# adelacvg/NS2VC

Measured on AMD Instinct MI355X. Metric: denoiser-steps/sec (10s@24kHz Vocos latent, bs32), higher is better.
Workload: dtype fp16

## Files before the change

### include/ns2vc_hip.h

```cpp
#ifndef NS2VC_HIP_H
#define NS2VC_HIP_H

#include <stddef.h>
#include <stdint.h>

#ifdef __cplusplus
extern "C" {
#endif

#define NS2VC_ABI_VERSION 7
#define NS2VC_MAX_LEVELS 8
#define NS2VC_NCOEF 12

typedef struct ns2vc_unet ns2vc_unet;

typedef struct ns2vc_unet_cfg {
  int32_t latent_channels;
  int32_t content_channels;
  int32_t n_levels;
  int32_t block_out_channels[NS2VC_MAX_LEVELS];
  int32_t norm_num_groups;
  int32_t cross_attention_dim;
  int32_t heads;
  int32_t layers_per_block;
// ... 133 lines not shown
int ns2vc_k_ffn(const ns2vc_ffn_args* a, int precision, void* stream);
size_t ns2vc_xattn_pack_bytes(int B, int Lk, int hd);
int ns2vc_k_xattn_pack(const void* k, int ldk, const void* v, int ldv, int B, int Lk, int hd, void* out, int precision, void* stream);

typedef struct ns2vc_geglu_args {
  const void* yn; int32_t ldy;
  const float* ln_stats; float ln_eps;
  const void* wstream; const float* consts;
  void* out_op; int32_t ldo;
  int32_t M, dim;
  unsigned* ln_health;
} ns2vc_geglu_args;
int ns2vc_pack_geglu(const float* w1_packed_host, const float* bias1_packed_host, int dim, int precision, void** out_stream_dev, float** out_consts_dev);
int ns2vc_k_geglu(const ns2vc_geglu_args* a, int precision, void* stream);
int ns2vc_pack_geglu_host(const float* w1_packed_host, const float* bias1_packed_host, int dim, int precision, uint16_t* stream_out, float* consts_out);

typedef struct ns2vc_rowchain_args {
  const void* a_op; int32_t lda;
  const void* wstream; const float* bias1; const float* consts2;
  const float* res; int32_t ldres;
  float* out1_f32; int32_t ldo1;
  void* out2_op; int32_t ldo2;
  float ln_eps; int32_t M, dim, n2;
  unsigned* ln_health;
  const float* gn_x; int32_t ldx;
  const long long* gn_stats; const float* gn_gamma; const float* gn_beta;
  float gn_eps; int32_t T, G;
  int32_t slices;
} ns2vc_rowchain_args;
int ns2vc_pack_rowchain(const float* w1_host, const float* w2_host, int dim, int n2, int precision, void** out_stream_dev);
// ... 36 lines not shown
```

### ns2vc_amd/_lib.py

```python
from __future__ import annotations

import ctypes as C
import os
from typing import Optional

_HERE = os.path.dirname(os.path.abspath(__file__))
LIB_PATH = os.path.join(_HERE, "lib", "libns2vc_hip.so")
NCOEF = 12
MAX_LEVELS = 8
PREC_F32, PREC_BF16, PREC_F16 = 0, 1, 2
ABI_VERSION = 7


class Ns2vcError(RuntimeError):
    pass


class UnetCfg(C.Structure):
    _fields_ = [
        ("latent_channels", C.c_int32), ("content_channels", C.c_int32), ("n_levels", C.c_int32),
        ("block_out_channels", C.c_int32 * MAX_LEVELS), ("norm_num_groups", C.c_int32),
        ("cross_attention_dim", C.c_int32), ("heads", C.c_int32), ("layers_per_block", C.c_int32),
        ("pool_heads", C.c_int32),
    ]
# ... 43 lines not shown
        ("pre_bias", C.c_void_p),
        ("pre_res", C.c_void_p), ("pre_ldres", C.c_int32),
        ("att_q", C.c_void_p), ("att_ldq", C.c_int32),
        ("att_kv", C.c_void_p), ("att_bias", C.c_void_p), ("att_scale", C.c_float), ("att_Lk", C.c_int32),
    ]


class GegluArgs(C.Structure):
    _fields_ = [
        ("yn", C.c_void_p), ("ldy", C.c_int32),
        ("ln_stats", C.c_void_p), ("ln_eps", C.c_float),
        ("wstream", C.c_void_p), ("consts", C.c_void_p),
        ("out_op", C.c_void_p), ("ldo", C.c_int32),
        ("M", C.c_int32), ("dim", C.c_int32),
        ("ln_health", C.c_void_p),
    ]


class RowchainArgs(C.Structure):
    _fields_ = [
        ("a_op", C.c_void_p), ("lda", C.c_int32),
        ("wstream", C.c_void_p), ("bias1", C.c_void_p), ("consts2", C.c_void_p),
        ("res", C.c_void_p), ("ldres", C.c_int32),
        ("out1_f32", C.c_void_p), ("ldo1", C.c_int32),
        ("out2_op", C.c_void_p), ("ldo2", C.c_int32),
        ("ln_eps", C.c_float), ("M", C.c_int32), ("dim", C.c_int32), ("n2", C.c_int32),
        ("ln_health", C.c_void_p),
        ("gn_x", C.c_void_p), ("ldx", C.c_int32),
        ("gn_stats", C.c_void_p), ("gn_gamma", C.c_void_p), ("gn_beta", C.c_void_p),
        ("gn_eps", C.c_float), ("T", C.c_int32), ("G", C.c_int32),
# ... 73 lines not shown
    "ns2vc_pack_conv3_tiled": (_I, [_P, _I, _I, _I, _I, _PP]),
    "ns2vc_weight_rowsum": (_I, [_P, _I, _I, _I, _PP]),
    "ns2vc_debug_set_gemm_trace": (_I, [_P]),
    "ns2vc_debug_set_gemm_tile": (_I, [_I, _I, _I]),
    "ns2vc_debug_placement": (_I, [_P, _I, _I, C.POINTER(C.c_uint32)]),
    "ns2vc_debug_poison": (_I, [C.c_uint, _I, _P]),
    "ns2vc_k_attention": (_I, [C.POINTER(AttnArgs), _I, _I, _P]),
    "ns2vc_pack_ffn": (_I, [_P, _P, _I, _I, _PP]),
    "ns2vc_pack_ffn_pre": (_I, [_P, _P, _P, _I, _I, _PP]),
    "ns2vc_xattn_pack_bytes": (C.c_size_t, [_I, _I, _I]),
    "ns2vc_k_xattn_pack": (_I, [_P, _I, _P, _I, _I, _I, _I, _P, _I, _P]),
    "ns2vc_k_ffn": (_I, [C.POINTER(FfnArgs), _I, _P]),
    "ns2vc_pack_geglu": (_I, [_P, _P, _I, _I, _PP, _PP]),
    "ns2vc_k_geglu": (_I, [C.POINTER(GegluArgs), _I, _P]),
    "ns2vc_pack_geglu_host": (_I, [_P, _P, _I, _I, _P, _P]),
    "ns2vc_debug_set_geglu_min_rows": (_I, [_I]),
    "ns2vc_pack_rowchain": (_I, [_P, _P, _I, _I, _I, _PP]),
    "ns2vc_pack_rowchain_sliced": (_I, [_P, _P, _I, _I, _I, _I, _PP]),
    "ns2vc_k_rowchain": (_I, [C.POINTER(RowchainArgs), _I, _P]),
    "ns2vc_debug_set_rowchain_tokens": (_I, [_I]),
    "ns2vc_debug_set_attn_keys": (_I, [_I]),
    "ns2vc_debug_set_attn_optimistic": (_I, [_I]),
    "ns2vc_k_groupnorm_stats": (_I, [_P, _I, _I, _P, _I, _I, _I, C.c_float, _P, _P, _P, _I, _I, _I, _P, _I, _P]),
    "ns2vc_k_groupnorm_stats2": (_I, [_P, _I, _I, _P, _P, _I, _I, _P, _I, _I, _I, C.c_float, _P, _P, _P, _I, _I, _I, _P, _P, _I, _P]),
    "ns2vc_k_groupnorm": (_I, [_P, _I, _I, _P, _I, _I, _I, _I, _I, C.c_float, _P, _P, _P, _I, _I, _I, _P, _P, _I, _P]),
    "ns2vc_k_layernorm_apply": (_I, [_P, _I, _I, _I, C.c_float, _P, _I, _P]),
    "ns2vc_to_operand": (_I, [_P, C.c_size_t, _I, _PP]),
    "ns2vc_from_operand": (_I, [_P, C.c_size_t, _I, _P]),
    "ns2vc_round_to_operand": (_I, [_P, C.c_size_t, _I, _P]),
    "ns2vc_k_nct_to_btc": (_I, [_P, _I, _I, _I, _P, _I, _I, _P]),
# ... 35 lines not shown
```

### ns2vc_amd/csrc/engine.cpp

```cpp
#include "common.h"

#include <algorithm>
#include <cmath>
#include <cstdarg>
#include <cstdio>
#include <cstring>
#include <cstdlib>
#include <functional>
#include <map>
#include <memory>
#include <string>
#include <vector>
#include <mutex>

using namespace ns2vc;

namespace ns2vc {
hipError_t pack_ffn_stream(const float* w1p, const float* w2f, const float* w0, int dim, int prec, std::vector<unsigned short>& out);
hipError_t pack_rowchain_stream(const float* w1, const float* w2, int dim, int n2, int prec, std::vector<unsigned short>& out, int slices = 1);
int rowchain_slice_blocks(int n2, int slices);
void set_ffn_trace(unsigned long long* p);
typedef ::ns2vc_geglu_args GegluArgs;
bool geglu_eligible(int dim, int T, int prec);
hipError_t pack_geglu_stream(const float* w1p, const float* bias1p, int dim, int prec, std::vector<unsigned short>& stream, std::vector<float>& consts);
hipError_t launch_geglu(const GegluArgs& a, int prec, hipStream_t s);
hipError_t init_geglu_attributes();
void set_rc_trace(unsigned long long* p);
void set_ts_trace(unsigned long long* p);
void set_gg_trace(unsigned long long* p);
void set_attn_optimistic(int on);
}

namespace {

int g_geglu_min_rows = 4608;

thread_local std::string g_err;

int fail(const char* fmt, ...) {
  char buf[1024];
  va_list ap;
// ... 31 lines not shown
  bool shortcut = false;
  float *n1g = nullptr, *n1b = nullptr, *n2g = nullptr, *n2b = nullptr;
  PackedW conv1, conv2, sc;
};
struct AttnW {
  std::string prefix;
  int dim = 0, kv_off = 0;
  float *ng = nullptr, *nb = nullptr;
  PackedW proj_in, qkv, o1, q2, o2, ff1, ff2, proj_out;
  PackedW ffpo;
  void* ffn_pre_stream = nullptr;
  void* ffn_stream = nullptr;
  float* ffn_consts = nullptr;
  void* geglu_stream = nullptr;
  float* geglu_consts = nullptr;
  void *chain_in = nullptr, *chain_mid = nullptr;
  void* chain_in_s2 = nullptr;
  float *chain_in_consts = nullptr, *chain_mid_consts = nullptr;
};
struct BlockW {
  std::string kind;
  int index = 0, level = 0, channels = 0;
  std::vector<ResnetW> res;
  std::vector<AttnW> attn;
  int sampler = 0;
  PackedW samp;
};

struct Op {
  std::string name;
// ... 555 lines not shown
          for (int r = 0; r < 8 * d; ++r) { cs[2 * r] = ws[r]; cs[2 * r + 1] = ff1_bias[r]; }
          a.ffn_consts = P.upload_f32(cs);
        } else {
          a.ffn_stream = nullptr; a.ffn_pre_stream = nullptr; a.ffn_consts = nullptr;
        }
        if (geglu_eligible(d, 1, h->prec)) {
          std::vector<unsigned short> st;
          std::vector<float> cs;
          if (pack_geglu_stream(ff1_rows.data(), ff1_bias.data(), d, h->prec, st, cs) != hipSuccess) return fail("geglu stream packing failed");
          void* dev = nullptr;
          if (hipMalloc(&dev, st.size() * 2) != hipSuccess) return fail("hipMalloc failed (weights)");
          h->weight_allocs.push_back(dev);
          if (hipMemcpy(dev, st.data(), st.size() * 2, hipMemcpyHostToDevice) != hipSuccess) return fail("hipMemcpy failed (weights)");
          a.geglu_stream = dev;
          a.geglu_consts = P.upload_f32(cs);
        }
      }
      {
        const HostTensor& wk = P.T(t + ".attn2.to_k.weight");
        const HostTensor& wv = P.T(t + ".attn2.to_v.weight");
        if (P.err) return 1;
        a.kv_off = kv_off;
        kv_rows.insert(kv_rows.end(), wk.data.begin(), wk.data.end());
        kv_rows.insert(kv_rows.end(), wv.data.begin(), wv.data.end());
        kv_off += 2 * d;
      }
    }
    if (b.sampler) {
      const std::string p = b.kind == "down" ? "down_blocks." + std::to_string(b.index) + ".downsamplers.0.conv"
                                             : "up_blocks." + std::to_string(b.index) + ".upsamplers.0.conv";
// ... 342 lines not shown
      f.B = B; f.T = Tl; f.M = M; f.dim = d; f.ln_health = h->ln_health;
      const double fl = 2.0 * M * (double)d * ((ffn_pre ? 14.0 : 13.0) * d) + (xatt ? 4.0 * B * h->cfg.heads * (double)Tl * Lp * hd : 0.0);
      add(a.prefix + (xatt ? ".ffn[attn2.sdpa+to_out+geglu+ff.out+proj_out]" : ffn_pre ? ".ffn[attn2.to_out+geglu+ff.out+proj_out]" : ".ffn[geglu+ff.out+proj_out]"),
          [=](hipStream_t s) { return launch_ffn(f, pr, s); }, 1, fl,
          (double)M * d * (opsz + 8.0 + (ffn_pre ? 4.0 : 0.0) + (out_op ? opsz : 0.0)) + (ffn_pre ? 14.0 : 13.0) * d * d * opsz +
              (xatt ? (double)opsz * B * d * 2.0 * Lp : 0.0));
      return;
    }
    if (!r3) layernorm(t + ".norm3");
    if (r3 && h->fuse_geglu && a.geglu_stream && geglu_eligible(d, Tl, pr) && M >= g_geglu_min_rows) {
      ns2vc_geglu_args f;
      memset(&f, 0, sizeof(f));
      f.yn = yn; f.ldy = d; f.ln_stats = r3; f.ln_eps = 1e-5f;
      f.wstream = a.geglu_stream; f.consts = a.geglu_consts;
      f.out_op = ffh; f.ldo = 4 * d; f.M = M; f.dim = d; f.ln_health = h->ln_health;
      add(t + ".ff.geglu[token-stationary]", [=](hipStream_t s) { return launch_geglu(f, pr, s); }, 1, 2.0 * M * (double)d * 8.0 * d,
          (double)M * d * opsz * 5.0 + (double)M * (d / 64) * 8.0 + 8.0 * d * d * opsz);
    } else {
      g = base(yn, d, d, Tl, Tl, a.ff1, nullptr, ffh, 4 * d);
      g.geglu = 1;
      consume(g, r3, a.ff1);
      gemm(t + ".ff.geglu", g);
    }
    if (fold) {
      g = base(ffh, 4 * d, 4 * d, Tl, Tl, a.ffpo, out, out_op, d);
      g.a2 = yraw; g.lda2 = d; g.c2 = d;
      g.res = x; g.ldres = d;
      g.stats = new_stats(out, Tl, d);
      gemm(a.prefix + ".ff.out+proj_out", g);
    } else {
// ... 1211 lines not shown
int ns2vc_pack_geglu_host(const float* w1_packed_host, const float* bias1_packed_host, int dim, int precision, uint16_t* stream_out, float* consts_out) {
  if (!w1_packed_host || !stream_out || !consts_out) return fail("null argument");
  std::vector<unsigned short> st;
  std::vector<float> cs;
  if (pack_geglu_stream(w1_packed_host, bias1_packed_host, dim, precision, st, cs) != hipSuccess) return fail("geglu: dim must be 384 and the precision 16-bit");
  memcpy(stream_out, st.data(), st.size() * 2);
  memcpy(consts_out, cs.data(), cs.size() * 4);
  return 0;
}
int ns2vc_k_geglu(const ns2vc_geglu_args* a, int precision, void* stream) {
  if (!a) return fail("null args");
  hipError_t e = launch_geglu(*a, precision, (hipStream_t)stream);
  if (e != hipSuccess) return fail("launch_geglu: %s", hipGetErrorString(e));
  return 0;
}
int ns2vc_k_attention(const ns2vc_attn_args* a, int head_dim, int precision, void* stream) {
  if (!a) return fail("null args");
  hipError_t e = launch_attention(*a, head_dim, precision, (hipStream_t)stream);
  if (e != hipSuccess) return fail("launch_attention: %s", hipGetErrorString(e));
  return 0;
}
int ns2vc_k_groupnorm(const float* a0, int lda0, int c0, const float* a1, int lda1, int c1, int B, int T, int G, float eps,
                      const float* gamma, const float* beta, const float* temb, int ldtemb, int temb_off, int silu, void* out_op,
                      void* raw_op, int precision, void* stream) {
  const int rows = 32, nchunk = (T + rows - 1) / rows;
  double* part = nullptr;
  HIPCHK(hipMalloc((void**)&part, (size_t)B * nchunk * G * 2 * sizeof(double)));
  hipError_t e = launch_gn_partial(a0, lda0, c0, a1, lda1, c1, B, T, G, part, nchunk, rows, (hipStream_t)stream);
  if (e == hipSuccess)
    e = launch_gn_apply(a0, lda0, c0, a1, lda1, c1, B, T, G, eps, part, nchunk, nullptr, nullptr, gamma, beta, temb, ldtemb, temb_off, silu,
// ... 77 lines not shown
```

### ns2vc_amd/csrc/geglu.hip

```cpp
#include "common.h"
#include "mma.h"
#include <type_traits>
#include <vector>

#ifndef NS2VC_GG_ABLATE
#define NS2VC_GG_ABLATE 0
#endif

#ifndef NS2VC_GEMM_TRACE
#define NS2VC_GEMM_TRACE 0
#endif
#ifndef NS2VC_GG_PRIO
#define NS2VC_GG_PRIO 0
#endif
#ifndef NS2VC_GG_ROTATE
#define NS2VC_GG_ROTATE 0
#endif
#ifndef NS2VC_GG_PINGPONG
#define NS2VC_GG_PINGPONG 1
#endif

namespace ns2vc {

typedef ::ns2vc_geglu_args GegluArgs;

__device__ unsigned long long* g_gg_trace = nullptr;
void set_gg_trace(unsigned long long* p) { (void)hipMemcpyToSymbol(HIP_SYMBOL(g_gg_trace), &p, sizeof(p)); }
#if NS2VC_GEMM_TRACE
#define GG_NOW() __builtin_readcyclecounter()
#define GG_ACC(i) do { const unsigned long long t_ = GG_NOW(); tacc[i] += t_ - tmark; tmark = t_; } while (0)
#else
#define GG_NOW() 0ull
#define GG_ACC(i) do {} while (0)
#endif

constexpr int GG_TILE = 128 * 128;
constexpr int GG_TOK = 128;
constexpr int GG_SPLIT = 4;
constexpr int GG_RING = 8;
// ... 6 lines not shown
  static constexpr int STAGE = 4 * 32 * 128;
  static constexpr int LDS = GG_RING * GG_TILE + CONSTS + STAGE;
  static_assert(LDS <= 160 * 1024, "LDS budget");
  static_assert((4 * D / 64) % GG_SPLIT == 0, "whole unit blocks per quarter");
  static_assert(KT % 2 == 0, "fragment double buffer: the parity of a step is the parity of its K tile");
  static_assert(NP >= GG_RING, "prologue issues a full ring");
};

static inline int gg_unit_of_row(int m) { return 16 * ((m >> 2) & 1) + 4 * (m >> 3) + (m & 3); }

template <int N> __device__ __forceinline__ void gg_wait_tiles(int t) {
  if constexpr (N == 0) wait_vmcnt<0>();
  else { if (t >= N) wait_vmcnt<2 * N>(); else gg_wait_tiles<N - 1>(t); }
}

template <typename TM, int D>
__global__ __launch_bounds__(512) void geglu_kernel(const GegluArgs a) {
  op_mode_init<TM>();
  using G = GegluGeom<D>;
  constexpr int KT = G::KT, UB = G::UB, NP = G::NP, RING = GG_RING;
  extern __shared__ __attribute__((aligned(16))) char smem[];
  char* const ring = smem;
  const float* const consts = reinterpret_cast<const float*>(smem + RING * GG_TILE);

  const int tid = threadIdx.x, lane = tid & 63;
  const int wave = __builtin_amdgcn_readfirstlane(tid >> 6);
  const int hg = wave & 1, tq = wave >> 1;
  unsigned long long tacc[8] = {0, 0, 0, 0, 0, 0, 0, 0}, tmark = 0;
  (void)tacc; (void)tmark;
  const unsigned long long t_entry = GG_NOW();
  (void)t_entry;
  const int l31 = lane & 31, hi = lane >> 5;
  const int sw = (l31 >> 1) & 7;
  const unsigned lds0 = (unsigned)(size_t)smem;

  const int ntb = (a.M + GG_TOK - 1) / GG_TOK;
  int tb, q;
  {
    const int nwg = ntb * GG_SPLIT, bid = blockIdx.x;
    const int qn = nwg >> 3, rn = nwg & 7, xcd = bid & 7, idx = bid >> 3;
    const int swz = (xcd < rn ? xcd * (qn + 1) : rn * (qn + 1) + (xcd - rn) * qn) + idx;
    tb = swz / GG_SPLIT;
    q = swz - tb * GG_SPLIT;
  }
  const int m0 = tb * GG_TOK;
  const int mtok = m0 + 32 * tq + l31;

  const i32x4_t rW = make_rsrc(a.wstream, (unsigned long long)GG_SPLIT * NP * GG_TILE);
  const unsigned lane16 = (unsigned)(lane * 16);
  const unsigned wq0 = (unsigned)(q * NP) * GG_TILE;
#if NS2VC_GG_ROTATE
  const int rot = __builtin_amdgcn_readfirstlane(tb % UB);
#else
  const int rot = 0;
#endif
  auto ubm = [&](int u) __attribute__((always_inline)) { const int v = u + rot; return v >= UB ? v - UB : v; };
  auto issue_tile = [&](int p, int slot) __attribute__((always_inline)) {
    const int u = p / KT, pt = ubm(u) * KT + (p - u * KT);
#pragma unroll
    for (int j = 0; j < 2; ++j) blds16(rW, lane16, wq0 + (unsigned)(pt * GG_TILE + (j * 8 + wave) * 1024), lds0 + slot * GG_TILE + (j * 8 + wave) * 1024);
  };
  constexpr int NT0 = RING - KT * GG_TOK * 128 / GG_TILE;
  static_assert(NT0 >= 1, "room for a first weight tile beside the token panel");
  constexpr int PANEL0 = NT0 * GG_TILE;
  static_assert(PANEL0 + KT * GG_TOK * 128 <= RING * GG_TILE, "the token panel fits in the ring slots it borrows");
// ... 64 lines not shown
    for (int kt = 0; kt < KT; ++kt)
#pragma unroll
      for (int ks = 0; ks < 4; ++ks) asm volatile("" : "+v"(tk[kt][ks]));
    asm volatile("s_waitcnt lgkmcnt(0)" ::: "memory");
    __builtin_amdgcn_s_barrier();
#pragma unroll
    for (int p0 = NT0; p0 < RING; ++p0) issue_tile(p0, p0);
  }
#if NS2VC_GG_PRIO
  if (wave >= 4) __builtin_amdgcn_s_setprio(1);
#endif
  const unsigned long long t_pro = GG_NOW();
  (void)t_pro;
  tmark = t_pro;

  int p = 0, slot = 0;
  f32x16_t av, ag, pv, pg;
  uint32_t hp[8];
#pragma unroll
  for (int r = 0; r < 16; ++r) { av[r] = 0.f; ag[r] = 0.f; pv[r] = 0.f; pg[r] = 0.f; }
#pragma unroll
  for (int r = 0; r < 8; ++r) hp[r] = 0u;

  auto chunk = [&](int ubp, int j) __attribute__((always_inline)) {
    const float* cv = consts + (size_t)(128 * ubm(ubp) + 64 * hg) * 2;
    const float4 v0 = *reinterpret_cast<const float4*>(cv + (8 * j + 4 * hi) * 2);
    const float4 v1 = *reinterpret_cast<const float4*>(cv + (8 * j + 4 * hi) * 2 + 4);
    const float4 g0 = *reinterpret_cast<const float4*>(cv + (32 + 8 * j + 4 * hi) * 2);
    const float4 g1 = *reinterpret_cast<const float4*>(cv + (32 + 8 * j + 4 * hi) * 2 + 4);
    const float wsv[4] = {v0.x, v0.z, v1.x, v1.z}, bv[4] = {v0.y, v0.w, v1.y, v1.w};
    const float wsg[4] = {g0.x, g0.z, g1.x, g1.z}, bg[4] = {g0.y, g0.w, g1.y, g1.w};
    float hh[4];
#pragma unroll
    for (int i = 0; i < 4; ++i) {
      const float xv = rstd * (pv[4 * j + i] - mean * wsv[i]) + bv[i];
      const float xg = rstd * (pg[4 * j + i] - mean * wsg[i]) + bg[i];
#if NS2VC_GG_ABLATE & 1
      hh[i] = xv + xg;
#else
      hh[i] = xv * gelu_erf_f(xg);
#endif
    }
    hp[2 * j] = Op16<TM>::pack(hh[0], hh[1]);
    hp[2 * j + 1] = Op16<TM>::pack(hh[2], hh[3]);
  };
  char* const stage = smem + RING * GG_TILE + G::CONSTS + tq * (32 * 128);
  const i32x4_t rO = uniform_rsrc(make_rsrc(a.out_op, (unsigned long long)a.M * (unsigned long long)a.ldo * 2ull));
  const int srow = 16 * hg + (lane >> 3);
  unsigned ooff[2];
#pragma unroll
  for (int j = 0; j < 2; ++j) {
    const int m = m0 + 32 * tq + srow + 8 * j;
    ooff[j] = m < a.M ? ((unsigned)m * (unsigned)a.ldo + (unsigned)(q * UB * 64)) * 2u + (unsigned)((lane & 7) * 16) : 0xC0000000u;
  }
  auto stage_block = [&]() __attribute__((always_inline)) {
    char* row = stage + l31 * 128;
    const int c0 = 4 * hg + 2 * hi, x = l31 & 7;
    const u32x4_t v0 = {hp[0], hp[1], hp[2], hp[3]}, v1 = {hp[4], hp[5], hp[6], hp[7]};
    *reinterpret_cast<u32x4_t*>(row + ((c0 ^ x) * 16)) = v0;
    *reinterpret_cast<u32x4_t*>(row + (((c0 + 1) ^ x) * 16)) = v1;
  };
  auto store_block = [&](int ubp) __attribute__((always_inline)) {
    const unsigned so = (unsigned)__builtin_amdgcn_readfirstlane(ubm(ubp) * 128);
    const u32x4_t v0 = *reinterpret_cast<const u32x4_t*>(stage + srow * 128 + (((lane & 7) ^ (srow & 7)) * 16));
    const u32x4_t v1 = *reinterpret_cast<const u32x4_t*>(stage + (srow + 8) * 128 + (((lane & 7) ^ (srow & 7)) * 16));
    asm volatile("buffer_store_dwordx4 %0, %1, %2, %3 offen " NS2VC_WT_MOD "\n\tbuffer_store_dwordx4 %4, %5, %2, %3 offen " NS2VC_WT_MOD "\n\ts_nop 1"
                 :: "v"(v0), "v"(ooff[0]), "s"(rO), "s"(so), "v"(v1), "v"(ooff[1]) : "memory");
  };
#if NS2VC_GG_PINGPONG
// ... 96 lines not shown
  for (int kt = 0; kt < KT; ++kt) step(T_{}, F_{}, kt, 0);
#pragma unroll 1
  for (int ub = 1; ub < UB; ++ub) {
#pragma unroll
    for (int r = 0; r < 16; ++r) { pv[r] = av[r]; pg[r] = ag[r]; av[r] = 0.f; ag[r] = 0.f; }
#pragma unroll
    for (int kt = 0; kt < KT; ++kt) step(T_{}, T_{}, kt, ub);
  }
#if NS2VC_GG_PINGPONG
  if (wave < 4) __builtin_amdgcn_s_barrier();
#endif
#pragma unroll
  for (int r = 0; r < 16; ++r) { pv[r] = av[r]; pg[r] = ag[r]; }
#pragma unroll
  for (int kt = 0; kt < 5; ++kt) step(F_{}, T_{}, kt, UB);
#if NS2VC_GEMM_TRACE
  if (g_gg_trace && lane == 0) {
    unsigned long long* tr = g_gg_trace + ((size_t)blockIdx.x * 8 + wave) * 16;
    tr[0] = t_entry; tr[1] = t_pro;
    for (int i = 0; i < 5; ++i) tr[2 + i] = tacc[i];
    tr[7] = GG_NOW();
    unsigned hwid;
    asm volatile("s_getreg_b32 %0, hwreg(HW_REG_HW_ID)" : "=s"(hwid));
    tr[8] = hwid;
  }
#endif
}

bool geglu_eligible(int dim, int T, int prec) { return dim == 384 && T >= 1 && (prec == PREC_BF16 || prec == PREC_F16); }

hipError_t pack_geglu_stream(const float* w1p, const float* bias1p, int dim, int prec, std::vector<unsigned short>& stream, std::vector<float>& consts) {
  if (dim != 384 || (prec != PREC_BF16 && prec != PREC_F16)) return hipErrorInvalidValue;
  const int KT = dim / 64, NUB = 4 * dim / 64;
  stream.clear();
  stream.reserve((size_t)8 * dim * dim);
  consts.assign((size_t)8 * dim * 2, 0.f);
  auto src_row = [&](int sr) {
    const int grp = sr >> 6, half = (sr >> 5) & 1, m = sr & 31;
    return grp * 64 + half * 32 + gg_unit_of_row(m);
  };
  for (int ubg = 0; ubg < NUB; ++ubg)
    for (int kt = 0; kt < KT; ++kt)
      for (int r = 0; r < 128; ++r) {
// ... 15 lines not shown

template <typename TM> static hipError_t launch_geglu_t(const GegluArgs& a, hipStream_t s) {
  const int ntb = (a.M + GG_TOK - 1) / GG_TOK;
  hipLaunchKernelGGL((geglu_kernel<TM, 384>), dim3(ntb * GG_SPLIT), dim3(512), GegluGeom<384>::LDS, s, a);
  return hipGetLastError();
}

hipError_t launch_geglu(const GegluArgs& a, int prec, hipStream_t s) {
  if (!geglu_eligible(a.dim, 1, prec) || a.M <= 0) return hipErrorInvalidValue;
  if (!a.yn || !a.ln_stats || !a.wstream || !a.consts || !a.out_op) return hipErrorInvalidValue;
  if (a.ldy < a.dim || a.ldo < 4 * a.dim || (a.ldy & 7) || (a.ldo & 7) || (unsigned long long)a.M * a.ldy * 2ull > 0xFFF00000ull || (unsigned long long)a.M * a.ldo * 2ull > 0x7FF00000ull) return hipErrorInvalidValue;
  if ((reinterpret_cast<uintptr_t>(a.out_op) & 15) != 0) return hipErrorInvalidValue;
  return prec == PREC_BF16 ? launch_geglu_t<bf16_t>(a, s) : launch_geglu_t<f16_t>(a, s);
}

hipError_t init_geglu_attributes() {
  hipError_t e = hipFuncSetAttribute(reinterpret_cast<const void*>(geglu_kernel<bf16_t, 384>), hipFuncAttributeMaxDynamicSharedMemorySize, (int)GegluGeom<384>::LDS);
  if (e == hipSuccess) e = hipFuncSetAttribute(reinterpret_cast<const void*>(geglu_kernel<f16_t, 384>), hipFuncAttributeMaxDynamicSharedMemorySize, (int)GegluGeom<384>::LDS);
  return e;
}

}
```

Before: 279.0.

## Fuse GEGLU, FF out and proj_out into one token-stationary kernel with inter-workgroup sync

```diff
diff --git a/include/ns2vc_hip.h b/include/ns2vc_hip.h
--- a/include/ns2vc_hip.h
+++ b/include/ns2vc_hip.h
@@ -171,6 +171,23 @@
 int ns2vc_pack_geglu(const float* w1_packed_host, const float* bias1_packed_host, int dim, int precision, void** out_stream_dev, float** out_consts_dev);
 int ns2vc_k_geglu(const ns2vc_geglu_args* a, int precision, void* stream);
 int ns2vc_pack_geglu_host(const float* w1_packed_host, const float* bias1_packed_host, int dim, int precision, uint16_t* stream_out, float* consts_out);
+
+typedef struct ns2vc_ffn384_args {
+  ns2vc_geglu_args gg;
+  const void* wstream;
+  const float* bias;
+  const float* res; int32_t ldres;
+  float* out_f32; int32_t ldo_f32;
+  void* out_op; int32_t ldo_op;
+  long long* stats;
+  int32_t T;
+  unsigned long long* sync;
+  unsigned* alone;
+  int32_t flags;
+} ns2vc_ffn384_args;
+int ns2vc_pack_ffn384(const float* w2f_host, int dim, int precision, void** out_stream_dev);
+int ns2vc_pack_ffn384_host(const float* w2f_host, int dim, int precision, uint16_t* stream_out);
+int ns2vc_k_ffn384(const ns2vc_ffn384_args* a, int precision, void* stream);
 
 typedef struct ns2vc_rowchain_args {
   const void* a_op; int32_t lda;
diff --git a/ns2vc_amd/_lib.py b/ns2vc_amd/_lib.py
--- a/ns2vc_amd/_lib.py
+++ b/ns2vc_amd/_lib.py
@@ -81,6 +81,22 @@
         ("out_op", C.c_void_p), ("ldo", C.c_int32),
         ("M", C.c_int32), ("dim", C.c_int32),
         ("ln_health", C.c_void_p),
+    ]
+
+
+class Ffn384Args(C.Structure):
+    _fields_ = [
+        ("gg", GegluArgs),
+        ("wstream", C.c_void_p),
+        ("bias", C.c_void_p),
+        ("res", C.c_void_p), ("ldres", C.c_int32),
+        ("out_f32", C.c_void_p), ("ldo_f32", C.c_int32),
+        ("out_op", C.c_void_p), ("ldo_op", C.c_int32),
+        ("stats", C.c_void_p),
+        ("T", C.c_int32),
+        ("sync", C.c_void_p),
+        ("alone", C.c_void_p),
+        ("flags", C.c_int32),
     ]
 
 
@@ -184,6 +200,9 @@
     "ns2vc_pack_geglu": (_I, [_P, _P, _I, _I, _PP, _PP]),
     "ns2vc_k_geglu": (_I, [C.POINTER(GegluArgs), _I, _P]),
     "ns2vc_pack_geglu_host": (_I, [_P, _P, _I, _I, _P, _P]),
+    "ns2vc_pack_ffn384": (_I, [_P, _I, _I, _PP]),
+    "ns2vc_pack_ffn384_host": (_I, [_P, _I, _I, _P]),
+    "ns2vc_k_ffn384": (_I, [C.POINTER(Ffn384Args), _I, _P]),
     "ns2vc_debug_set_geglu_min_rows": (_I, [_I]),
     "ns2vc_pack_rowchain": (_I, [_P, _P, _I, _I, _I, _PP]),
     "ns2vc_pack_rowchain_sliced": (_I, [_P, _P, _I, _I, _I, _I, _PP]),
diff --git a/ns2vc_amd/csrc/engine.cpp b/ns2vc_amd/csrc/engine.cpp
--- a/ns2vc_amd/csrc/engine.cpp
+++ b/ns2vc_amd/csrc/engine.cpp
@@ -25,6 +25,8 @@
 hipError_t pack_geglu_stream(const float* w1p, const float* bias1p, int dim, int prec, std::vector<unsigned short>& stream, std::vector<float>& consts);
 hipError_t launch_geglu(const GegluArgs& a, int prec, hipStream_t s);
 hipError_t init_geglu_attributes();
+hipError_t pack_ffn384_stream(const float* w2f, int dim, int prec, std::vector<unsigned short>& out);
+hipError_t launch_ffn384(const ns2vc_ffn384_args& f, int prec, hipStream_t s);
 void set_rc_trace(unsigned long long* p);
 void set_ts_trace(unsigned long long* p);
 void set_gg_trace(unsigned long long* p);
@@ -86,6 +88,7 @@
   float* ffn_consts = nullptr;
   void* geglu_stream = nullptr;
   float* geglu_consts = nullptr;
+  void* ffn384_stream = nullptr;
   void *chain_in = nullptr, *chain_mid = nullptr;
   void* chain_in_s2 = nullptr;
   float *chain_in_consts = nullptr, *chain_mid_consts = nullptr;
@@ -671,6 +674,11 @@
           if (hipMemcpy(dev, st.data(), st.size() * 2, hipMemcpyHostToDevice) != hipSuccess) return fail("hipMemcpy failed (weights)");
           a.geglu_stream = dev;
           a.geglu_consts = P.upload_f32(cs);
+          if (pack_ffn384_stream(rows.data(), d, h->prec, st) != hipSuccess) return fail("ffn384 stream packing failed");
+          if (hipMalloc(&dev, st.size() * 2) != hipSuccess) return fail("hipMalloc failed (weights)");
+          h->weight_allocs.push_back(dev);
+          if (hipMemcpy(dev, st.data(), st.size() * 2, hipMemcpyHostToDevice) != hipSuccess) return fail("hipMemcpy failed (weights)");
+          a.ffn384_stream = dev;
         }
       }
       {
@@ -1043,6 +1051,28 @@
       f.yn = yn; f.ldy = d; f.ln_stats = r3; f.ln_eps = 1e-5f;
       f.wstream = a.geglu_stream; f.consts = a.geglu_consts;
       f.out_op = ffh; f.ldo = 4 * d; f.M = M; f.dim = d; f.ln_health = h->ln_health;
+      const int ntb = (M + 127) / 128;
+      unsigned* words = (fold && a.ffn384_stream && Tl >= 128 && M >= 4608 && 32 * ((ntb + 7) / 8) <= h->cus) ? new_sync(ntb) : nullptr;
+      if (words) {
+        ns2vc_ffn384_args ff;
+        memset(&ff, 0, sizeof(ff));
+        ff.gg = f;
+        ff.wstream = a.ffn384_stream; ff.bias = a.ffpo.bias;
+        ff.res = x; ff.ldres = d;
+        ff.out_f32 = out; ff.ldo_f32 = d; ff.out_op = out_op; ff.ldo_op = d;
+        ff.stats = new_stats(out, Tl, d);
+        ff.T = Tl;
+        ff.sync = reinterpret_cast<unsigned long long*>(words);
+        ff.alone = h->ln_health ? h->ln_health + 52 : nullptr;
+        add(a.prefix + ".ffn[geglu+ff.out+proj_out][token-stationary]", [=](hipStream_t s) { return launch_ffn384(ff, pr, s); }, 1,
+            2.0 * M * (double)d * 13.0 * d,
+            (double)M * d * (opsz * 5.0 + 4.0 + 4.0 + (out_op ? opsz : 0.0)) + (double)M * (d / 64) * 8.0 + 13.0 * d * d * opsz);
+        if (!sizing) {
+          const size_t nbytes = (size_t)ntb * 8;
+          ops->back().rearm = [=](hipStream_t s) { return launch_zero(words, (nbytes + 15) & ~(size_t)15, s); };
+        }
+        return;
+      }
       add(t + ".ff.geglu[token-stationary]", [=](hipStream_t s) { return launch_geglu(f, pr, s); }, 1, 2.0 * M * (double)d * 8.0 * d,
           (double)M * d * opsz * 5.0 + (double)M * (d / 64) * 8.0 + 8.0 * d * d * opsz);
     } else {
@@ -2284,6 +2314,31 @@
   if (e != hipSuccess) return fail("launch_geglu: %s", hipGetErrorString(e));
   return 0;
 }
+int ns2vc_pack_ffn384(const float* w2f_host, int dim, int precision, void** out_stream_dev) {
+  if (!w2f_host || !out_stream_dev) return fail("null argument");
+  hipError_t e = init_geglu_attributes();
+  if (e != hipSuccess) return fail("kernel attribute setup failed: %s", hipGetErrorString(e));
+  std::vector<unsigned short> st;
+  if (pack_ffn384_stream(w2f_host, dim, precision, st) != hipSuccess) return fail("ffn384: dim must be 384 and the precision 16-bit");
+  void* d = nullptr;
+  HIPCHK(hipMalloc(&d, st.size() * 2));
+  HIPCHK(hipMemcpy(d, st.data(), st.size() * 2, hipMemcpyHostToDevice));
+  *out_stream_dev = d;
+  return 0;
+}
+int ns2vc_pack_ffn384_host(const float* w2f_host, int dim, int precision, uint16_t* stream_out) {
+  if (!w2f_host || !stream_out) return fail("null argument");
+  std::vector<unsigned short> st;
+  if (pack_ffn384_stream(w2f_host, dim, precision, st) != hipSuccess) return fail("ffn384: dim must be 384 and the precision 16-bit");
+  memcpy(stream_out, st.data(), st.size() * 2);
+  return 0;
+}
+int ns2vc_k_ffn384(const ns2vc_ffn384_args* a, int precision, void* stream) {
+  if (!a) return fail("null args");
+  hipError_t e = launch_ffn384(*a, precision, (hipStream_t)stream);
+  if (e != hipSuccess) return fail("launch_ffn384: %s", hipGetErrorString(e));
+  return 0;
+}
 int ns2vc_k_attention(const ns2vc_attn_args* a, int head_dim, int precision, void* stream) {
   if (!a) return fail("null args");
   hipError_t e = launch_attention(*a, head_dim, precision, (hipStream_t)stream);
diff --git a/ns2vc_amd/csrc/geglu.hip b/ns2vc_amd/csrc/geglu.hip
--- a/ns2vc_amd/csrc/geglu.hip
+++ b/ns2vc_amd/csrc/geglu.hip
@@ -16,6 +16,9 @@
 #ifndef NS2VC_GG_ROTATE
 #define NS2VC_GG_ROTATE 0
 #endif
+#ifndef NS2VC_FF4_SPIN
+#define NS2VC_FF4_SPIN 256
+#endif
 #ifndef NS2VC_GG_PINGPONG
 #define NS2VC_GG_PINGPONG 1
 #endif
@@ -23,6 +26,7 @@
 namespace ns2vc {
 
 typedef ::ns2vc_geglu_args GegluArgs;
+typedef ::ns2vc_ffn384_args Ffn384Args;
 
 __device__ unsigned long long* g_gg_trace = nullptr;
 void set_gg_trace(unsigned long long* p) { (void)hipMemcpyToSymbol(HIP_SYMBOL(g_gg_trace), &p, sizeof(p)); }
@@ -59,8 +63,13 @@
   else { if (t >= N) wait_vmcnt<2 * N>(); else gg_wait_tiles<N - 1>(t); }
 }
 
-template <typename TM, int D>
-__global__ __launch_bounds__(512) void geglu_kernel(const GegluArgs a) {
+static __device__ __forceinline__ const GegluArgs& gg_of(const GegluArgs& a) { return a; }
+static __device__ __forceinline__ const GegluArgs& gg_of(const Ffn384Args& f) { return f.gg; }
+template <typename TM, int D> __device__ __forceinline__ void ffn384_phase3(const Ffn384Args& f, int tb, int q, const u32x4_t (&tk)[D / 64][4]);
+
+template <typename TM, int D, bool FF, typename AT>
+__device__ __forceinline__ void geglu_body(const AT& args) {
+  const GegluArgs& a = gg_of(args);
   op_mode_init<TM>();
   using G = GegluGeom<D>;
   constexpr int KT = G::KT, UB = G::UB, NP = G::NP, RING = GG_RING;
@@ -81,7 +90,14 @@
 
   const int ntb = (a.M + GG_TOK - 1) / GG_TOK;
   int tb, q;
-  {
+  if constexpr (FF) {
+    const int bid = blockIdx.x, cls = bid & 7, idx = bid >> 3;
+    const int base = ntb >> 3, rem = ntb & 7;
+    const int nb = base + (cls < rem ? 1 : 0), b0 = cls * base + min(cls, rem);
+    if (idx / GG_SPLIT >= nb) return;
+    tb = b0 + idx / GG_SPLIT;
+    q = idx % GG_SPLIT;
+  } else {
     const int nwg = ntb * GG_SPLIT, bid = blockIdx.x;
     const int qn = nwg >> 3, rn = nwg & 7, xcd = bid & 7, idx = bid >> 3;
     const int swz = (xcd < rn ? xcd * (qn + 1) : rn * (qn + 1) + (xcd - rn) * qn) + idx;
@@ -93,7 +109,7 @@
 
   const i32x4_t rW = make_rsrc(a.wstream, (unsigned long long)GG_SPLIT * NP * GG_TILE);
   const unsigned lane16 = (unsigned)(lane * 16);
-  const unsigned wq0 = (unsigned)(q * NP) * GG_TILE;
+  unsigned wq0 = (unsigned)(q * NP) * GG_TILE;
 #if NS2VC_GG_ROTATE
   const int rot = __builtin_amdgcn_readfirstlane(tb % UB);
 #else
@@ -188,6 +204,16 @@
   (void)t_pro;
   tmark = t_pro;
 
+  char* const stage = smem + RING * GG_TILE + G::CONSTS + tq * (32 * 128);
+  const i32x4_t rO = uniform_rsrc(make_rsrc(a.out_op, (unsigned long long)a.M * (unsigned long long)a.ldo * 2ull));
+  const int srow = 16 * hg + (lane >> 3);
+  unsigned ooff[2];
+#pragma unroll
+  for (int j = 0; j < 2; ++j) {
+    const int m = m0 + 32 * tq + srow + 8 * j;
+    ooff[j] = m < a.M ? ((unsigned)m * (unsigned)a.ldo + (unsigned)(q * UB * 64)) * 2u + (unsigned)((lane & 7) * 16) : 0xC0000000u;
+  }
+  auto sweep = [&]() __attribute__((always_inline)) {
   int p = 0, slot = 0;
   f32x16_t av, ag, pv, pg;
   uint32_t hp[8];
@@ -218,15 +244,6 @@
     hp[2 * j] = Op16<TM>::pack(hh[0], hh[1]);
     hp[2 * j + 1] = Op16<TM>::pack(hh[2], hh[3]);
   };
-  char* const stage = smem + RING * GG_TILE + G::CONSTS + tq * (32 * 128);
-  const i32x4_t rO = uniform_rsrc(make_rsrc(a.out_op, (unsigned long long)a.M * (unsigned long long)a.ldo * 2ull));
-  const int srow = 16 * hg + (lane >> 3);
-  unsigned ooff[2];
-#pragma unroll
-  for (int j = 0; j < 2; ++j) {
-    const int m = m0 + 32 * tq + srow + 8 * j;
-    ooff[j] = m < a.M ? ((unsigned)m * (unsigned)a.ldo + (unsigned)(q * UB * 64)) * 2u + (unsigned)((lane & 7) * 16) : 0xC0000000u;
-  }
   auto stage_block = [&]() __attribute__((always_inline)) {
     char* row = stage + l31 * 128;
     const int c0 = 4 * hg + 2 * hi, x = l31 & 7;
@@ -353,6 +370,67 @@
   for (int r = 0; r < 16; ++r) { pv[r] = av[r]; pg[r] = ag[r]; }
 #pragma unroll
   for (int kt = 0; kt < 5; ++kt) step(F_{}, T_{}, kt, UB);
+  };
+  sweep();
+  if constexpr (FF) {
+    const Ffn384Args& f = args;
+    asm volatile("s_waitcnt vmcnt(0)" ::: "memory");
+    __syncthreads();
+    int* const okf = reinterpret_cast<int*>(smem + G::LDS - 16);
+    if (tid == 0) {
+      unsigned xcc;
+      asm volatile("s_getreg_b32 %0, hwreg(HW_REG_XCC_ID)" : "=s"(xcc));
+      xcc &= 7u;
+      unsigned long long* const cnt = f.sync + tb;
+      const unsigned long long inc = 1ull | (1ull << (16 + 4 * xcc));
+      const unsigned long long want = (unsigned long long)GG_SPLIT | ((unsigned long long)GG_SPLIT << (16 + 4 * xcc));
+      const unsigned long long mine = 0xffffull | (0xfull << (16 + 4 * xcc));
+      unsigned long long old, v, zero = 0ull;
+      asm volatile("global_atomic_add_x2 %0, %1, %2, off sc0\n\ts_waitcnt vmcnt(0)" : "=&v"(old) : "v"(cnt), "v"(inc) : "memory");
+      v = old + inc;
+      int ok = v == want;
+      bool hopeless = (f.flags & 1) || (old >> 62) != 0 || (v & 0xffffull) > (unsigned)GG_SPLIT || (v & ~mine) != 0;
+      for (int it = 0; !ok && !hopeless && it < NS2VC_FF4_SPIN; ++it) {
+        asm volatile("global_atomic_add_x2 %0, %1, %2, off sc0\n\ts_waitcnt vmcnt(0)" : "=&v"(v) : "v"(cnt), "v"(zero) : "memory");
+        ok = v == want;
+        hopeless = (v & 0xffffull) > (unsigned)GG_SPLIT || (v & ~mine) != 0;
+        if (!ok && !hopeless) __builtin_amdgcn_s_sleep(2);
+      }
+      okf[0] = ok && !(f.flags & 1);
+    }
+    __syncthreads();
+    if (!okf[0]) {
+      if (tid == 0 && f.alone) atomicAdd(f.alone, 1u);
+      const int q_own = q;
+#pragma unroll 1
+      for (int qq = 0; qq < GG_SPLIT; ++qq) {
+        if (qq == q_own) continue;
+        q = qq;
+        wq0 = (unsigned)(q * NP) * GG_TILE;
+#pragma unroll
+        for (int j = 0; j < 2; ++j) {
+          const int m = m0 + 32 * tq + srow + 8 * j;
+          ooff[j] = m < a.M ? ((unsigned)m * (unsigned)a.ldo + (unsigned)(q * UB * 64)) * 2u + (unsigned)((lane & 7) * 16) : 0xC0000000u;
+        }
+        __syncthreads();
+        const i32x4_t rC = make_rsrc(a.consts, (unsigned long long)GG_SPLIT * G::CONSTS);
+#pragma unroll
+        for (int j = 0; j < (G::CONSTS + 8191) / 8192; ++j) {
+          const unsigned off = (unsigned)((j * 8 + wave) * 1024);
+          if (off < (unsigned)G::CONSTS) blds16(rC, lane16, (unsigned)(q * G::CONSTS) + off, lds0 + RING * GG_TILE + off);
+        }
+#pragma unroll
+        for (int p0 = 0; p0 < RING; ++p0) issue_tile(p0, p0);
+        wait_vmcnt<0>();
+        __builtin_amdgcn_s_barrier();
+        sweep();
+        asm volatile("s_waitcnt vmcnt(0)" ::: "memory");
+      }
+      q = q_own;
+    }
+    __syncthreads();
+    ffn384_phase3<TM, D>(f, tb, q, tk);
+  }
 #if NS2VC_GEMM_TRACE
   if (g_gg_trace && lane == 0) {
     unsigned long long* tr = g_gg_trace + ((size_t)blockIdx.x * 8 + wave) * 16;
@@ -366,6 +444,209 @@
 #endif
 }
 
+template <typename TM, int D>
+__global__ __launch_bounds__(512) void geglu_kernel(const GegluArgs a) { geglu_body<TM, D, false>(a); }
+
+constexpr int F3_ROWS = 96;
+constexpr int F3_WT = F3_ROWS * 128;
+constexpr int F3_SLOT = F3_WT + GG_TILE;
+constexpr int F3_RING = 5;
+template <int D> struct F3Geom {
+  static constexpr int KT = D / 64;
+  static constexpr int YS = KT / 2;
+  static constexpr int HT = 4 * D / 64;
+  static constexpr int NS = YS + HT;
+  static constexpr int QBYTES = (KT + HT) * F3_WT;
+  static constexpr int PITCH = F3_ROWS + 4;
+  static constexpr int RED = 2 * 128 * PITCH * 4;
+  static_assert(D == 4 * F3_ROWS, "a quarter of the channels per workgroup");
+  static_assert(F3_RING * F3_SLOT <= GegluGeom<D>::LDS - 16, "the ring fits in the sweep's LDS (its last 16 bytes hold the seam flag)");
+  static_assert(RED + 8 * 24 * 4 <= F3_RING * F3_SLOT, "epilogue staging fits in the ring");
+  static_assert(KT % 2 == 0 && 2 * F3_WT == 24 * 1024, "a y stage is 24 pieces of 1 KB: three per wave");
+};
+template <int N> __device__ __forceinline__ void f3_wait_le(int c) {
+  if constexpr (N == 0) wait_vmcnt<0>();
+  else { if (c >= N) wait_vmcnt<N>(); else f3_wait_le<N - 1>(c); }
+}
+
+template <typename TM, int D>
+__device__ __forceinline__ void ffn384_phase3(const Ffn384Args& f, int tb, int q, const u32x4_t (&tk)[D / 64][4]) {
+  using F = F3Geom<D>;
+  constexpr int NS = F::NS, YS = F::YS;
+  const GegluArgs& a = f.gg;
+  extern __shared__ __attribute__((aligned(16))) char smem[];
+  const int tid = threadIdx.x, lane = tid & 63;
+  const int wave = __builtin_amdgcn_readfirstlane(tid >> 6);
+  const int tq = wave >> 1, kh = wave & 1;
+  const int l31 = lane & 31, hi = lane >> 5, sw = (l31 >> 1) & 7;
+  const unsigned lds0 = (unsigned)(size_t)smem, lane16 = (unsigned)(lane * 16);
+  const int m0 = tb * GG_TOK;
+  const bool lo4 = wave < 4;
+  const i32x4_t rW = make_rsrc(f.wstream, 4ull * F::QBYTES);
+  const i32x4_t rH = make_rsrc(a.out_op, (unsigned long long)a.M * a.ldo * 2ull);
+  const unsigned wq = (unsigned)(q * F::QBYTES);
+  unsigned hv[3];
+#pragma unroll
+  for (int j = 0; j < 3; ++j) {
+    const int pc = lo4 ? wave : 4 + 3 * (wave - 4) + j;
+    const int prow = 8 * pc + (lane >> 3), m = m0 + prow;
+    hv[j] = m < a.M ? (unsigned)m * (unsigned)a.ldo * 2u + (unsigned)(((lane & 7) ^ ((prow >> 1) & 7)) * 16) : DMA_OOB;
+  }
+  auto issue = [&](int s) __attribute__((always_inline)) {
+    const unsigned sb = lds0 + (unsigned)((s % F3_RING) * F3_SLOT);
+    if (s < YS) {
+#pragma unroll
+      for (int j = 0; j < 3; ++j) blds16(rW, lane16, wq + (unsigned)(s * 2 * F3_WT + (wave + 8 * j) * 1024), sb + (wave + 8 * j) * 1024);
+    } else {
+      const int kt = s - YS;
+      const unsigned wo = wq + (unsigned)(YS * 2 * F3_WT + kt * F3_WT);
+      blds16(rW, lane16, wo + wave * 1024, sb + wave * 1024);
+      if (lo4) {
+        blds16(rW, lane16, wo + (wave + 8) * 1024, sb + (wave + 8) * 1024);
+        blds16(rH, hv[0], (unsigned)(kt * 128), sb + F3_WT + wave * 1024);
+      } else {
+#pragma unroll
+        for (int j = 0; j < 3; ++j) blds16(rH, hv[j], (unsigned)(kt * 128), sb + F3_WT + (4 + 3 * (wave - 4) + j) * 1024);
+      }
+    }
+  };
+  auto wait_stage = [&](int s) __attribute__((always_inline)) {
+    const int last = min(s + F3_RING - 1, NS - 1);
+    int c = 0;
+    for (int u = s + 1; u <= last; ++u) c += (u < YS || lo4) ? 3 : 4;
+    f3_wait_le<4 * (F3_RING - 1)>(c);
+    __builtin_amdgcn_s_barrier();
+    return smem + (s % F3_RING) * F3_SLOT;
+  };
+  auto refill = [&](int s) __attribute__((always_inline)) {
+    asm volatile("s_waitcnt lgkmcnt(0)" ::: "memory");
+    __builtin_amdgcn_s_barrier();
+    if (s + F3_RING < NS) issue(s + F3_RING);
+  };
+#pragma unroll
+  for (int s = 0; s < F3_RING; ++s) issue(s);
+
+  f32x16_t acc[3];
+#pragma unroll
+  for (int i = 0; i < 3; ++i)
+#pragma unroll
+    for (int r = 0; r < 16; ++r) acc[i][r] = 0.f;
+  auto yseg = [&](auto khc) __attribute__((always_inline)) {
+    constexpr int KH = decltype(khc)::value;
+#pragma unroll
+    for (int s = 0; s < YS; ++s) {
+      const char* T = wait_stage(s);
+#pragma unroll
+      for (int t = 0; t < 2; ++t) {
+        const int kt = 2 * s + t;
+        u32x4_t fa[3][2];
+#pragma unroll
+        for (int s2 = 0; s2 < 2; ++s2) {
+          const int c = ((2 * (2 * KH + s2) + hi) ^ sw) * 16;
+#pragma unroll
+          for (int i = 0; i < 3; ++i) fa[i][s2] = *reinterpret_cast<const u32x4_t*>(T + t * F3_WT + (32 * i + l31) * 128 + c);
+        }
+        if (t == 1) refill(s);
+        else asm volatile("s_waitcnt lgkmcnt(0)" ::: "memory");
+#pragma unroll
+        for (int s2 = 0; s2 < 2; ++s2)
+#pragma unroll
+          for (int i = 0; i < 3; ++i) MmaT<TM>::mma(acc[i], fa[i][s2], tk[kt][2 * KH + s2]);
+      }
+    }
+  };
+  if (kh) yseg(std::integral_constant<int, 1>{});
+  else yseg(std::integral_constant<int, 0>{});
+  const int hrow = (32 * tq + l31) * 128;
+#pragma unroll 2
+  for (int s = YS; s < NS; ++s) {
+    const char* T = wait_stage(s);
+    u32x4_t fa[3][2], fb[2];
+#pragma unroll
+    for (int s2 = 0; s2 < 2; ++s2) {
+      const int c = ((2 * (2 * kh + s2) + hi) ^ sw) * 16;
+      fb[s2] = *reinterpret_cast<const u32x4_t*>(T + F3_WT + hrow + c);
+#pragma unroll
+      for (int i = 0; i < 3; ++i) fa[i][s2] = *reinterpret_cast<const u32x4_t*>(T + (32 * i + l31) * 128 + c);
+    }
+    refill(s);
+#pragma unroll
+    for (int s2 = 0; s2 < 2; ++s2)
+#pragma unroll
+      for (int i = 0; i < 3; ++i) MmaT<TM>::mma(acc[i], fa[i][s2], fb[s2]);
+  }
+
+  const int etok = tid >> 2, part = tid & 3;
+  const int em = m0 + etok;
+  const bool eok = em < a.M;
+  float4 rr[6];
+#pragma unroll
+  for (int j = 0; j < 6; ++j) {
+    const int n = F3_ROWS * q + 4 * (part + 4 * j);
+    rr[j] = eok ? *reinterpret_cast<const float4*>(f.res + (size_t)em * f.ldres + n) : make_float4(0.f, 0.f, 0.f, 0.f);
+    const float4 bb = *reinterpret_cast<const float4*>(f.bias + n);
+    rr[j].x += bb.x; rr[j].y += bb.y; rr[j].z += bb.z; rr[j].w += bb.w;
+  }
+  lds_barrier();
+  float* const E = reinterpret_cast<float*>(smem);
+  {
+    float* const ew = E + (kh * 128 + 32 * tq + l31) * F::PITCH + 4 * hi;
+#pragma unroll
+    for (int i = 0; i < 3; ++i)
+#pragma unroll
+      for (int j = 0; j < 4; ++j) *reinterpret_cast<float4*>(ew + 32 * i + 8 * j) = make_float4(acc[i][4 * j], acc[i][4 * j + 1], acc[i][4 * j + 2], acc[i][4 * j + 3]);
+  }
+  lds_barrier();
+  const int b0 = min(m0, a.M - 1) / f.T;
+  const int mB = (b0 + 1) * f.T;
+  float sm[2][6], sq[2][6];
+  TM* const oo = reinterpret_cast<TM*>(f.out_op);
+#pragma unroll
+  for (int j = 0; j < 6; ++j) {
+    const int cq = part + 4 * j, n = F3_ROWS * q + 4 * cq;
+    const float4 e0 = *reinterpret_cast<const float4*>(E + etok * F::PITCH + 4 * cq);
+    const float4 e1 = *reinterpret_cast<const float4*>(E + (128 + etok) * F::PITCH + 4 * cq);
+    float4 v;
+    v.x = (e0.x + e1.x) + rr[j].x; v.y = (e0.y + e1.y) + rr[j].y; v.z = (e0.z + e1.z) + rr[j].z; v.w = (e0.w + e1.w) + rr[j].w;
+    float ps = 0.f, pq = 0.f;
+    if (eok) {
+      if (f.out_f32) out_f4(f.out_f32 + (size_t)em * f.ldo_f32 + n, v.x, v.y, v.z, v.w);
+      if (oo) out_op4<TM>(oo + (size_t)em * f.ldo_op + n, v.x, v.y, v.z, v.w);
+      ps = (v.x + v.y) + (v.z + v.w); pq = (v.x * v.x + v.y * v.y) + (v.z * v.z + v.w * v.w);
+    }
+    const bool second = em >= mB;
+    sm[0][j] = second ? 0.f : ps; sq[0][j] = second ? 0.f : pq;
+    sm[1][j] = second ? ps : 0.f; sq[1][j] = second ? pq : 0.f;
+  }
+  if (f.stats) {
+#pragma unroll
+    for (int o = 1; o < 64; o <<= 1)
+#pragma unroll
+      for (int j = 0; j < 6; ++j)
+#pragma unroll
+        for (int b = 0; b < 2; ++b) { sm[b][j] += __shfl_xor(sm[b][j], o); sq[b][j] += __shfl_xor(sq[b][j], o); }
+    float* const red = reinterpret_cast<float*>(smem + F::RED);
+    if (lane == 0)
+#pragma unroll
+      for (int b = 0; b < 2; ++b)
+#pragma unroll
+        for (int j = 0; j < 6; ++j) { red[wave * 24 + (b * 6 + j) * 2] = sm[b][j]; red[wave * 24 + (b * 6 + j) * 2 + 1] = sq[b][j]; }
+    lds_barrier();
+    if (tid < 24) {
+      const int b = tid / 12, j = (tid >> 1) % 6, mo = tid & 1;
+      float v = 0.f;
+      for (int w = 0; w < 8; ++w) v += red[w * 24 + tid];
+      if (b == 0 || (mB < a.M && mB < m0 + GG_TOK)) {
+        unsigned long long* st = reinterpret_cast<unsigned long long*>(f.stats) + ((size_t)(b0 + b) * (D / 16) + (F3_ROWS / 16) * q + j) * 2 + mo;
+        atomicAdd(st, (unsigned long long)llrint((double)v * (mo ? GN_SQ_SCALE : GN_SUM_SCALE)));
+      }
+    }
+  }
+}
+
+template <typename TM>
+__global__ __launch_bounds__(512) void ffn384_kernel(const Ffn384Args f) { geglu_body<TM, 384, true>(f); }
+
 bool geglu_eligible(int dim, int T, int prec) { return dim == 384 && T >= 1 && (prec == PREC_BF16 || prec == PREC_F16); }
 
 hipError_t pack_geglu_stream(const float* w1p, const float* bias1p, int dim, int prec, std::vector<unsigned short>& stream, std::vector<float>& consts) {
@@ -411,9 +692,46 @@
   return prec == PREC_BF16 ? launch_geglu_t<bf16_t>(a, s) : launch_geglu_t<f16_t>(a, s);
 }
 
+hipError_t pack_ffn384_stream(const float* w2f, int dim, int prec, std::vector<unsigned short>& out) {
+  if (dim != 384 || (prec != PREC_BF16 && prec != PREC_F16)) return hipErrorInvalidValue;
+  const size_t K = 5 * (size_t)dim;
+  out.clear();
+  out.reserve(K * dim);
+  auto tile = [&](int row0, int col0) {
+    for (int r = 0; r < F3_ROWS; ++r)
+      for (int pos = 0; pos < 8; ++pos) {
+        const int lc = pos ^ ((r >> 1) & 7);
+        for (int e = 0; e < 8; ++e) out.push_back(f32_to_op16_bits(w2f[(size_t)(row0 + r) * K + col0 + lc * 8 + e], prec));
+      }
+  };
+  for (int q = 0; q < GG_SPLIT; ++q) {
+    for (int kt = 0; kt < dim / 64; ++kt) tile(F3_ROWS * q, 4 * dim + 64 * kt);
+    for (int kt = 0; kt < 4 * dim / 64; ++kt) tile(F3_ROWS * q, 64 * kt);
+  }
+  return hipSuccess;
+}
+
+hipError_t launch_ffn384(const Ffn384Args& f, int prec, hipStream_t s) {
+  const GegluArgs& a = f.gg;
+  if (!geglu_eligible(a.dim, 1, prec) || a.M <= 0 || f.T < GG_TOK) return hipErrorInvalidValue;
+  if (!a.yn || !a.ln_stats || !a.wstream || !a.consts || !a.out_op || !f.wstream || !f.bias || !f.res || !f.sync || (!f.out_f32 && !f.out_op))
+    return hipErrorInvalidValue;
+  if (a.ldy < a.dim || a.ldo < 4 * a.dim || (a.ldy & 7) || (a.ldo & 7) || (unsigned long long)a.M * a.ldy * 2ull > 0xFFF00000ull || (unsigned long long)a.M * a.ldo * 2ull > 0x7FF00000ull) return hipErrorInvalidValue;
+  if (f.ldres < a.dim || (f.ldres & 3) || (f.out_f32 && (f.ldo_f32 < a.dim || (f.ldo_f32 & 3))) || (f.out_op && (f.ldo_op < a.dim || (f.ldo_op & 3)))) return hipErrorInvalidValue;
+  if (((reinterpret_cast<uintptr_t>(a.out_op) | reinterpret_cast<uintptr_t>(f.res) | reinterpret_cast<uintptr_t>(f.bias) | reinterpret_cast<uintptr_t>(f.out_f32)) & 15) ||
+      (reinterpret_cast<uintptr_t>(f.out_op) & 7) || (reinterpret_cast<uintptr_t>(f.sync) & 7))
+    return hipErrorInvalidValue;
+  const int nwg = 8 * GG_SPLIT * ((a.M + 8 * GG_TOK - 1) / (8 * GG_TOK));
+  if (prec == PREC_BF16) hipLaunchKernelGGL(ffn384_kernel<bf16_t>, dim3(nwg), dim3(512), GegluGeom<384>::LDS, s, f);
+  else hipLaunchKernelGGL(ffn384_kernel<f16_t>, dim3(nwg), dim3(512), GegluGeom<384>::LDS, s, f);
+  return hipGetLastError();
+}
+
 hipError_t init_geglu_attributes() {
   hipError_t e = hipFuncSetAttribute(reinterpret_cast<const void*>(geglu_kernel<bf16_t, 384>), hipFuncAttributeMaxDynamicSharedMemorySize, (int)GegluGeom<384>::LDS);
   if (e == hipSuccess) e = hipFuncSetAttribute(reinterpret_cast<const void*>(geglu_kernel<f16_t, 384>), hipFuncAttributeMaxDynamicSharedMemorySize, (int)GegluGeom<384>::LDS);
+  if (e == hipSuccess) e = hipFuncSetAttribute(reinterpret_cast<const void*>(ffn384_kernel<bf16_t>), hipFuncAttributeMaxDynamicSharedMemorySize, (int)GegluGeom<384>::LDS);
+  if (e == hipSuccess) e = hipFuncSetAttribute(reinterpret_cast<const void*>(ffn384_kernel<f16_t>), hipFuncAttributeMaxDynamicSharedMemorySize, (int)GegluGeom<384>::LDS);
   return e;
 }
 
```

New measurement: 278.9 (median of 6 runs). No clear change (-0.0%).
